# Tonanguyxiro/FastBN

Hardware: AMD Instinct MI355X
Metric: JT test-cases/sec (ALARM, Munin) + PC-stable CI-tests/sec, 1/2/4/8 GPU (higher is better)
Workload: dtype f64

## Files before the change

### fastbn_amd/csrc/jt_codegen.cpp

```cpp
#include <algorithm>
#include <map>
#include <cstdio>
#include <cstdlib>
#include <functional>
#include <sstream>
#include <string>

#include "fbn_internal.h"

namespace fbn {

namespace {

int LocOfT(const Table &t, int v) {
    for (size_t i = 0; i < t.vars.size(); ++i)
        if (t.vars[i] == v) return (int)i;
    return -1;
}

std::string Lit(double x) {
    char b[64];
    snprintf(b, sizeof b, "%.17g", x);
    std::string s = b;
    if (s.find_first_of(".eEn") == std::string::npos) s += ".0";
    return s;
}

}

bool JTCodegenEligible(const JTPlanHost &plan, int64_t *entry_ops) {
    int64_t tmax = 0, ops = 0;
    for (const auto &t : plan.cliques) {
        tmax = std::max<int64_t>(tmax, t.size());
        ops += t.size() * (4 + (int64_t)t.vars.size());
    }
    if (entry_ops) *entry_ops = ops;
    for (int d : plan.dom)
        if (d > 32) return false;
    return tmax <= 256 && ops <= 40000;
}

namespace {

class JTGen {
  public:
    JTGen(const JTPlanHost &p, bool fast_order, bool var_major) : plan(p), fast(fast_order), vmajor(var_major) {}
    int Run(std::string &src, int64_t *wave_entries, std::vector<double> &initv);
    int64_t lds_rows = 0;
    int64_t pool_rows = 0;
    JTPlacement place;
    bool iv_lds = false;

  private:
    const JTPlanHost &plan;
    const bool fast;
    const bool vmajor;
    std::ostringstream o;
    std::vector<int> okw_word, okw_pos, out_off;
    std::vector<int64_t> sep_row, init_off;
    std::vector<std::vector<int>> cand;
    std::vector<int> home;
    std::vector<int> msep;
    std::vector<int> mclq;
    void MargTerms(int v, const std::vector<std::vector<std::string>> &terms);
    int nobs = 0;
    bool profile = false;
    static constexpr int64_t kInitBatch = 16;
    bool in_merged = false;
    int min_waves = 1;
    bool marg_v2 = true;
    std::vector<std::vector<std::string>> col_loc, dis_loc;
    std::vector<bool> md_reg;
    std::vector<bool> leaf_rc, col_store;
    void LoadCol(const std::string &name, int s) {
        if (!leaf_rc[s]) return Load(name, s);
        const int c = plan.sep_down[s];
        const int64_t Ts = plan.seps[s].size(), Q = plan.cliques[c].size() / Ts;
        for (int64_t j = 0; j < Ts; ++j) o << "        double " << name << s << "_" << j << ";\n";
        o << "        { // recompute the Collect message of leaf clique " << c << "\n";
        const std::string P = "r" + name;
        InitProd(P, c, {}, -1, "");
        for (int64_t j = 0; j < Ts; ++j) {
            std::vector<std::string> terms;
            for (int64_t q = 0; q < Q; ++q) terms.push_back(N(P, c, q * Ts + j));
            o << "        " << name << s << "_" << j << " = " << TreeSum(terms) << ";\n";
        }
        o << "        }\n";
    }
    void PlaceMessages(const std::vector<int> &post, const std::vector<int> &pre, int64_t budget, int64_t reg_cap,
                       bool quiet);
    static constexpr int64_t kRegFile = 256, kRegSlackVM = 16, kRegSlackCM = 32, kDefaultRegPool = kRegFile;
    int64_t peak_need = 0;
    std::vector<int64_t> reg_extra;
    std::vector<std::string> reg_names;
    std::string B(int k) const {
        return profile ? "        FBN_OP_BOUNDARY(); FBN_STAMP(" + std::to_string(k) + ");\n" : "        FBN_OP_BOUNDARY();\n";
    }

    std::string R(int c) const {
        std::vector<unsigned> m(nobs, 0u);
        for (int v : plan.cliques[c].vars) m[v / 32] |= 1u << (v % 32);
        std::ostringstream t;
        t << "(" << plan.cliques[c].vars.size();
        for (int k = 0; k < nobs; ++k)
            if (m[k]) t << " - __builtin_popcount(obs" << k << " & " << m[k] << "u)";
        t << ")";
        return t.str();
    }
    std::string observed(int v) const {
        std::ostringstream t;
        t << "((obs" << v / 32 << " >> " << v % 32 << ") & 1u)";
        return t.str();
    }
    int child(int s) const { return plan.sep_down[s]; }
    int64_t SepIndex(const Table &t, const Table &sp, int64_t e) const {
        int64_t r = e, idx = 0;
        for (size_t j = 0; j < t.vars.size(); ++j) {
            const int64_t dgt = r / t.cum[j];
            r %= t.cum[j];
            const int l = LocOfT(sp, t.vars[j]);
            if (l >= 0) idx += dgt * sp.cum[l];
        }
        return idx;
    }
    void Init(const std::string &P, int c);
    void InitProd(const std::string &P, int c, const std::vector<std::pair<int, std::string>> &kids, int up,
                  const std::string &upM);
    void Mul(const std::string &P, int c, int s, const std::string &M);
    void SepCol(const std::string &P, int c, int s, bool store);
    void DMul(const std::string &P, int c, int s, const std::string &M);
    void SepDis(const std::string &P, int c, int s, const std::string &old, bool store);
    void Marg(const std::string &P, int c);
    void Load(const std::string &name, int s) {
        const auto &loc = name == "ld" ? dis_loc[s] : col_loc[s];
        for (int64_t j = 0; j < plan.seps[s].size(); ++j)
            o << "        const double " << name << s << "_" << j << " = " << loc[j] << ";\n";
    }
    static constexpr int64_t kRegEntries = 144;
    std::string N(const std::string &P, int c, int64_t e) const {
        if (e >= kRegEntries) return "L(" + std::to_string(e - kRegEntries) + ")";
        return P + std::to_string(c) + "_" + std::to_string(e);
    }
    bool normed = false;
    std::string Val(const std::string &P, int c, int64_t e) const {
        return (normed || fast) ? N(P, c, e) : "dv(" + N(P, c, e) + ", den, y)";
    }
    static std::string TreeSum(const std::vector<std::string> &t, size_t b, size_t e) {
        if (e - b == 1) return t[b];
        const size_t m = b + (e - b) / 2;
        return "(" + TreeSum(t, b, m) + " + " + TreeSum(t, m, e) + ")";
    }
    static std::string TreeSum(const std::vector<std::string> &t) { return TreeSum(t, 0, t.size()); }
    void Normalize(const std::string &P, int c) {
        const Table &t = plan.cliques[c];
        for (int64_t e = 0; e < t.size(); ++e) o << (e % 8 ? " " : (e ? "\n        " : "        ")) << N(P, c, e) << " = dv(" << N(P, c, e) << ", den, y);";
        o << "\n" << B(6);
        normed = true;
    }
};

void JTGen::Init(const std::string &P, int c) {
    const Table &t = plan.cliques[c];
    const int nv = (int)t.vars.size();
    std::vector<bool> ev_here(nv, true);
    for (int j = 0; j < nv; ++j) ev_here[j] = !fast || home[t.vars[j]] == c;
    for (int j = 0; j < nv; ++j) {
        const int v = t.vars[j];
        if (!ev_here[j]) continue;
        for (int d = 0; d < plan.dom[v]; ++d)
            o << (d ? " " : "        ") << "const bool k" << P << c << "_" << j << "_" << d << " = (okw" << okw_word[v] << " >> "
              << okw_pos[v] + d << ") & 1u;";
        o << "\n";
    }
    if (!fast) o << "        double s_" << P << c << " = 0.0;\n";
    const int64_t kB = 16, T = t.size();
    auto loads = [&](int64_t b0) {
        if (b0 >= T) return;
        o << "       ";
        for (int64_t e = b0; e < std::min(T, b0 + kB); ++e)
            o << " const double w" << P << c << "_" << e << " = IV(" << init_off[c] + e << ");";
        o << "\n        __builtin_amdgcn_sched_barrier(0);\n";
    };
    loads(0);
    for (int64_t b0 = 0; b0 < T; b0 += kB) {
        loads(b0 + kB);
        for (int64_t e = b0; e < std::min(T, b0 + kB); ++e) {
            std::ostringstream cond;
            int64_t r = e;
            bool any = false;
            for (int j = 0; j < nv; ++j) {
                const int64_t dgt = r / t.cum[j];
                r %= t.cum[j];
                if (!ev_here[j]) continue;
                cond << (any ? " && " : "") << "k" << P << c << "_" << j << "_" << dgt;
                any = true;
            }
            o << "        " << (e < kRegEntries ? "double " : "") << N(P, c, e) << " = ";
            if (any) o << "sel(" << cond.str() << ", w" << P << c << "_" << e << ");";
            else o << "w" << P << c << "_" << e << ";";
            if (!fast) o << " s_" << P << c << " += " << N(P, c, e) << ";";
            o << "\n";
        }
        o << "        __builtin_amdgcn_sched_barrier(0);\n";
    }
    if (!fast) o << "        den = s_" << P << c << "; y = 1.0 / den; bad |= den_bad(den);\n";
    o << B(2);
    normed = false;
}

void JTGen::InitProd(const std::string &P, int c, const std::vector<std::pair<int, std::string>> &kids, int up,
                     const std::string &upM) {
    const Table &t = plan.cliques[c];
    const int nv = (int)t.vars.size();
    std::vector<bool> ev_here(nv, false);
    for (int j = 0; j < nv; ++j) ev_here[j] = home[t.vars[j]] == c;
    for (int j = 0; j < nv; ++j) {
        if (!ev_here[j]) continue;
        const int v = t.vars[j];
        for (int d = 0; d < plan.dom[v]; ++d)
            o << (d ? " " : "        ") << "const double i" << P << c << "_" << j << "_" << d << " = (double)((okw"
              << okw_word[v] << " >> " << okw_pos[v] + d << ") & 1u);";
        o << "\n";
    }
    std::vector<std::vector<int64_t>> kidx(kids.size());
    for (size_t i = 0; i < kids.size(); ++i) {
        const Table &sp = plan.seps[kids[i].first];
        for (int64_t e = 0; e < t.size(); ++e) kidx[i].push_back(SepIndex(t, sp, e));
    }
    const int64_t Tup = up >= 0 ? plan.seps[up].size() : 0;
    const int64_t kB = kInitBatch, T = t.size();
    auto loads = [&](int64_t b0) {
        if (b0 >= T) return;
        o << "       ";
        for (int64_t e = b0; e < std::min(T, b0 + kB); ++e)
            o << " const double w" << P << c << "_" << e << " = IV(" << init_off[c] + e << ");";
        o << "\n        __builtin_amdgcn_sched_barrier(0);\n";
    };
    loads(0);
    for (int64_t b0 = 0; b0 < T; b0 += kB) {
        loads(b0 + kB);
        for (int64_t e = b0; e < std::min(T, b0 + kB); ++e) {
            std::vector<std::string> f{"w" + P + std::to_string(c) + "_" + std::to_string(e)};
            int64_t r = e;
            for (int j = 0; j < nv; ++j) {
                const int64_t dgt = r / t.cum[j];
                r %= t.cum[j];
                if (ev_here[j]) f.push_back("i" + P + std::to_string(c) + "_" + std::to_string(j) + "_" + std::to_string(dgt));
            }
            for (size_t i = 0; i < kids.size(); ++i)
                f.push_back(kids[i].second + std::to_string(kids[i].first) + "_" + std::to_string(kidx[i][e]));
            if (up >= 0) f.push_back(upM + std::to_string(up) + "_" + std::to_string(e % Tup));
            std::function<std::string(size_t, size_t)> prod = [&](size_t lo, size_t hi) -> std::string {
                if (hi - lo == 1) return f[lo];
                const size_t m = lo + (hi - lo) / 2;
                return "(" + prod(lo, m) + " * " + prod(m, hi) + ")";
            };
            o << "        " << (e < kRegEntries ? "double " : "") << N(P, c, e) << " = " << prod(0, f.size()) << ";\n";
        }
        o << "        __builtin_amdgcn_sched_barrier(0);\n";
    }
    o << B(2);
    normed = false;
}

void JTGen::Mul(const std::string &P, int c, int s, const std::string &M) {
    const Table &t = plan.cliques[c], &sp = plan.seps[s];
    std::vector<std::vector<int64_t>> inv(sp.size());
    for (int64_t e = 0; e < t.size(); ++e) inv[SepIndex(t, sp, e)].push_back(e);
    for (int64_t j = 0; j < sp.size(); ++j) {
        o << "       ";
        for (int64_t e : inv[j]) o << " " << N(P, c, e) << " = " << Val(P, c, e) << " * " << M << s << "_" << j << ";";
        o << "\n";
    }
    if (!fast) {
        o << "        { double sm = 0.0;";
        for (int64_t e = 0; e < t.size(); ++e) o << " sm += " << N(P, c, e) << ";";
        o << " den = sm; y = 1.0 / den; bad |= den_bad(den); }\n";
    }
    o << B(3);
    normed = false;
}

void JTGen::SepCol(const std::string &P, int c, int s, bool store) {
    const Table &t = plan.cliques[c];
    const int64_t Ts = plan.seps[s].size(), Q = t.size() / Ts;
    if (fast) {
        for (int64_t j = 0; j < Ts; ++j) {
            std::vector<std::string> terms;
            for (int64_t q = 0; q < Q; ++q) terms.push_back(N(P, c, q * Ts + j));
            o << "        const double mc" << s << "_" << j << " = " << TreeSum(terms) << ";";
            if (store) o << " " << col_loc[s][j] << " = mc" << s << "_" << j << ";";
            o << "\n";
        }
        if (!in_merged) o << B(4);
        return;
    }
    for (int64_t j = 0; j < Ts; ++j) {
        o << "        const double mc" << s << "_" << j << " = " << Val(P, c, j);
        for (int64_t q = 1; q < Q; ++q) o << " + " << Val(P, c, q * Ts + j);
        o << ";";
        if (store) o << " " << col_loc[s][j] << " = mc" << s << "_" << j << ";";
        o << "\n";
    }
    o << B(4);
}

void JTGen::DMul(const std::string &P, int c, int s, const std::string &M) {
    const Table &t = plan.cliques[c];
    const int64_t Ts = plan.seps[s].size();
    for (int64_t j = 0; j < Ts; ++j) {
        o << "       ";
        for (int64_t e = j; e < t.size(); e += Ts)
            o << " " << N(P, c, e) << " = " << Val(P, c, e) << " * " << M << s << "_" << j << ";";
        o << "\n";
    }
    if (!fast) {
        o << "        { double sm = 0.0;";
        for (int64_t e = 0; e < t.size(); ++e) o << " sm += " << N(P, c, e) << ";";
        o << " den = sm; y = 1.0 / den; bad |= den_bad(den); }\n";
    }
    o << B(5);
    normed = false;
}

void JTGen::SepDis(const std::string &P, int c, int s, const std::string &old, bool store) {
    const Table &t = plan.cliques[c], &sp = plan.seps[s];
    std::vector<std::vector<int64_t>> lists(sp.size());
    for (int64_t e = 0; e < t.size(); ++e) lists[SepIndex(t, sp, e)].push_back(e);
    if (fast) {
        for (int64_t j = 0; j < sp.size(); ++j) {
            std::vector<std::string> terms;
            for (int64_t e : lists[j]) terms.push_back(N(P, c, e));
            const std::string sa = "sa" + std::to_string(s) + "_" + std::to_string(j);
            o << "        const double " << sa << " = " << TreeSum(terms) << ";";
            o << " double md" << s << "_" << j << "; { const double od = " << old << s << "_" << j
              << "; const double q = " << sa << " * frcp(od); md" << s << "_" << j << " = (od == 0.0) ? 0.0 : q; }";
            if (store) o << " " << dis_loc[s][j] << " = md" << s << "_" << j << ";";
            o << "\n";
        }
        for (size_t l = 0; l < sp.vars.size(); ++l) {
            const int v = sp.vars[l];
            if (msep[v] != s) continue;
            std::vector<std::vector<std::string>> terms(plan.dom[v]);
            for (int64_t j = 0; j < sp.size(); ++j)
                terms[(j / sp.cum[l]) % sp.dims[l]].push_back("sa" + std::to_string(s) + "_" + std::to_string(j));
            MargTerms(v, terms);
        }
        if (!in_merged) o << B(7);
        return;
    }
    for (int64_t j = 0; j < sp.size(); ++j) {
        o << "        double md" << s << "_" << j << ";";
        o << " { double a = " << Val(P, c, lists[j][0]) << ";";
        for (size_t q = 1; q < lists[j].size(); ++q) o << " a += " << Val(P, c, lists[j][q]) << ";";
        o << " const double od = " << old << s << "_" << j << "; md" << s << "_" << j << " = (od == 0.0) ? 0.0 : a / od; }";
        if (store) o << " " << dis_loc[s][j] << " = md" << s << "_" << j << ";";
        o << "\n";
    }
    o << B(7);
}

void JTGen::MargTerms(int v, const std::vector<std::vector<std::string>> &terms) {
    const int dim = plan.dom[v];
    if (marg_v2) {
        o << "        { // marginal of var " << v << "\n          const bool ob = " << observed(v) << " != 0u;\n";
        std::vector<std::string> ps;
        for (int d = 0; d < dim; ++d) {
            o << "          const double p" << d << " = " << TreeSum(terms[d]) << ";\n";
            ps.push_back("p" + std::to_string(d));
        }
        o << "          const double tot = " << TreeSum(ps) << "; const double yt = frcp(tot); bad |= ob ? 0u : den_bad(tot);\n";
        if (v == 0) {
            o << "          if (ACT && !ob) { int lab = 0; double mp = 0.0, m2 = 0.0;";
            for (int d = 0; d < dim; ++d)
                o << " { const double q = dv(p" << d << ", tot, yt); if (q > mp) { m2 = mp; mp = q; lab = " << d
                  << "; } else if (q > m2) m2 = q; }";
            o << " labels[CS] = lab; bad |= (mp - m2 <= 1e-12 * mp) ? 1u : 0u; }\n";
        }
        for (int d = 0; d < dim; ++d) {
            const int64_t k = out_off[v] + d;
            if (marg_v2 && d + 1 < dim) {
                o << "          if (ACT) OUTS2(" << k << ", ob ? 0.0 : dv(p" << d << ", tot, yt), ob ? 0.0 : dv(p" << d + 1 << ", tot, yt));\n";
                ++d;
            } else {
                o << "          if (ACT) OUTS(" << k << ", ob ? 0.0 : dv(p" << d << ", tot, yt));\n";
            }
        }
        o << "        }\n";
        return;
    }
    o << "        if (!" << observed(v) << ") { // marginal of var " << v << "\n";
    std::vector<std::string> ps;
    for (int d = 0; d < dim; ++d) {
        o << "          const double p" << d << " = " << TreeSum(terms[d]) << ";\n";
        ps.push_back("p" + std::to_string(d));
    }
    o << "          const double tot = " << TreeSum(ps) << "; const double yt = frcp(tot); bad |= den_bad(tot);\n";
    if (v == 0) {
        o << "          if (ACT) { int lab = 0; double mp = 0.0, m2 = 0.0;";
        for (int d = 0; d < dim; ++d)
            o << " { const double q = dv(p" << d << ", tot, yt); if (q > mp) { m2 = mp; mp = q; lab = " << d
              << "; } else if (q > m2) m2 = q; }";
        o << " labels[CS] = lab; bad |= (mp - m2 <= 1e-12 * mp) ? 1u : 0u; }\n";
    }
    o << "          if (ACT) {";
    for (int d = 0; d < dim; ++d) o << " OUTS(" << out_off[v] + d << ", dv(p" << d << ", tot, yt));";
    o << " }\n        }\n";
}

void JTGen::Marg(const std::string &P, int c) {
    const Table &t = plan.cliques[c];
    for (size_t j = 0; j < t.vars.size(); ++j) {
        const int v = t.vars[j];
        const int dim = plan.dom[v];
        const int64_t cum = t.cum[j], bw = dim * cum, nhi = t.size() / bw;
        if (fast) {
            if (mclq[v] != c || msep[v] >= 0) continue;
            std::vector<std::vector<std::string>> terms(dim);
            for (int d = 0; d < dim; ++d)
                for (int64_t hi = 0; hi < nhi; ++hi)
                    for (int64_t l = 0; l < cum; ++l) terms[d].push_back(N(P, c, hi * bw + d * cum + l));
            MargTerms(v, terms);
            if (!in_merged) o << B(8);
            continue;
        } else {
            o << "        { int b = " << R(cand[v][0]) << ", sl = " << cand[v][0] << ";";
            for (size_t k = 1; k < cand[v].size(); ++k)
                o << " { const int r = " << R(cand[v][k]) << "; if (r < b) { b = r; sl = " << cand[v][k] << "; } }";
            o << "\n        if (sl == " << c << " && !" << observed(v) << ") { // marginal of var " << v << "\n";
        }
        if (fast) {
            std::vector<std::string> ps;
            for (int d = 0; d < dim; ++d) {
                std::vector<std::string> terms;
                for (int64_t hi = 0; hi < nhi; ++hi)
                    for (int64_t l = 0; l < cum; ++l) terms.push_back(N(P, c, hi * bw + d * cum + l));
                o << "          const double p" << d << " = " << TreeSum(terms) << ";\n";
                ps.push_back("p" + std::to_string(d));
            }
            o << "          const double tot = " << TreeSum(ps) << "; const double yt = frcp(tot); bad |= den_bad(tot);\n";
// ... 182 lines not shown
    for (int i : byst) {
        const Item &it = items[i];
        for (size_t k = 0; k < active.size();) {
            if (items[active[k]].b < it.a) {
                for (int64_t r : rows_of[active[k]]) free_rows.push_back(r);
                std::sort(free_rows.rbegin(), free_rows.rend());
                active.erase(active.begin() + k);
            } else {
                ++k;
            }
        }
        for (int64_t j = nreg[i]; j < it.n; ++j) {
            rows_of[i].push_back(free_rows.back());
            pool_rows = std::max<int64_t>(pool_rows, free_rows.back() + 1);
            free_rows.pop_back();
        }
        active.push_back(i);
    }
    col_loc.assign(ns, {});
    dis_loc.assign(ns, {});
    sep_row.assign(ns, -1);
    reg_names.clear();
    std::vector<int64_t> sep_skip(ns, 0);
    for (int s = 0; s < ns; ++s) sep_skip[s] = plan.seps[s].size();
    for (size_t i = 0; i < items.size(); ++i)
        if (!in_lds[i]) sep_skip[items[i].s] = std::min(sep_skip[items[i].s], nreg[i]);
    int64_t grow = 0;
    place = JTPlacement();
    for (size_t i = 0; i < items.size(); ++i) {
        const Item &it = items[i];
        auto &loc = it.dist ? dis_loc[it.s] : col_loc[it.s];
        loc.assign(it.n, std::string());
        for (int64_t j = 0; j < nreg[i]; ++j) {
            loc[j] = (it.dist ? "rd" : "rc") + std::to_string(it.s) + "_" + std::to_string(j);
            reg_names.push_back(loc[j]);
        }
        place.reg[it.dist] += nreg[i];
        if (in_lds[i]) {
            for (int64_t j = nreg[i]; j < it.n; ++j) loc[j] = "LP(" + std::to_string(rows_of[i][j - nreg[i]]) + ")";
            place.lds[it.dist] += it.n - nreg[i];
            continue;
        }
        if (nreg[i] == it.n) continue;
        if (sep_row[it.s] < 0) sep_row[it.s] = grow, grow += it.n - sep_skip[it.s];
        for (int64_t j = nreg[i]; j < it.n; ++j) loc[j] = "W(" + std::to_string(sep_row[it.s] + j - sep_skip[it.s]) + "LL)";
        place.global[it.dist] += it.n - nreg[i];
    }
    place.workspace_rows = grow;
    place.lds_pool_rows = pool_rows;
    for (int s = 0; s < ns; ++s) {
        if (sep_row[s] < 0) sep_row[s] = 0;
        if (dis_loc[s].empty()) dis_loc[s].assign(plan.seps[s].size(), "0.0");
        if (col_loc[s].empty()) col_loc[s].assign(plan.seps[s].size(), "0.0");
    }
    if (!quiet && KnobSet("FBN_JT_PLACE_DEBUG")) {
        int64_t leaf = 0;
        for (int s = 0; s < ns; ++s)
            if (plan.clique_down[plan.sep_down[s]].empty()) leaf += plan.seps[s].size();
        fprintf(stderr, "placement: pool %lld of %lld rows; Collect rows LDS %lld global %lld; Distribute rows LDS %lld "
                        "global %lld (registers: the rest); global rows %lld; leaf-separator rows %lld\n",
                (long long)pool_rows, (long long)cap, (long long)place.lds[0], (long long)place.global[0],
                (long long)place.lds[1], (long long)place.global[1], (long long)grow, (long long)leaf);
        if (reg_cap > 0)
            fprintf(stderr, "register pool (cap %lld rows): Collect rows %lld, Distribute rows %lld\n", (long long)reg_cap,
                    (long long)place.reg[0], (long long)place.reg[1]);
        std::string u;
        for (int t = 0; t <= 2 * nc; ++t) u += std::to_string(use[t]) + (t == nc - 1 ? " | " : " ");
        fprintf(stderr, "pool rows in use by time (Collect | Distribute): %s\n", u.c_str());
        if (fast) {
            std::string m;
            for (int v = 0; v < (int)plan.dom.size(); ++v) {
                const int t = msep[v] >= 0 ? nc + pi[plan.sep_up[msep[v]]] : nc + pi[mclq[v]];
                m += std::to_string(v) + ":" + std::to_string(t) + " ";
            }
            fprintf(stderr, "marginal time per variable: %s\n", m.c_str());
        }
    }
}

int JTGen::Run(std::string &src, int64_t *wave_entries, std::vector<double> &initv) {
    const int nc = (int)plan.cliques.size(), ns = (int)plan.seps.size(), V = plan.num_nodes;
    profile = KnobOr("FBN_JT_PROFILE", 0) != 0;
    marg_v2 = fast && KnobOr("FBN_JT_MARG_V2", 1) != 0;
    lds_rows = 0;
    for (const auto &t : plan.cliques) lds_rows = std::max<int64_t>(lds_rows, t.size() - kRegEntries);
    initv.clear();
    init_off.assign(nc, 0);
    for (int c = 0; c < nc; ++c) {
        init_off[c] = (int64_t)initv.size();
        initv.insert(initv.end(), plan.cliques[c].pot.begin(), plan.cliques[c].pot.end());
    }
    int SD = 0;
    out_off.assign(V, 0);
    for (int v = 0; v < V; ++v) out_off[v] = SD, SD += plan.dom[v];
    cand.assign(V, {});
    for (int c = 0; c < nc; ++c)
        for (int v : plan.cliques[c].vars) cand[v].push_back(c);
    home.assign(V, -1);
    for (int v = 0; v < V; ++v)
        for (int q : cand[v])
            if (home[v] < 0 || plan.cliques[q].size() < plan.cliques[home[v]].size()) home[v] = q;
    msep.assign(V, -1);
    if (fast)
        for (int sp = 0; sp < ns; ++sp)
            for (int v : plan.seps[sp].vars) {
                const int64_t have = msep[v] >= 0 ? plan.seps[msep[v]].size() : plan.cliques[home[v]].size();
                if (plan.seps[sp].size() < have) msep[v] = sp;
            }
    mclq = home;
    std::vector<int64_t> weight(nc, 0);
    {
        std::function<int64_t(int)> w = [&](int c) {
            weight[c] = plan.cliques[c].size();
            for (int s : plan.clique_down[c]) weight[c] += w(child(s));
            return weight[c];
        };
        for (int r : plan.roots) w(r);
    }
    auto dfs = [&](bool collect, int visit, std::vector<int> &post_o, std::vector<int> &pre_o) {
        std::vector<std::vector<int>> kids(nc);
        for (int c = 0; c < nc; ++c) {
            kids[c] = plan.clique_down[c];
            if (visit)
                std::stable_sort(kids[c].begin(), kids[c].end(), [&](int x, int y) {
                    return visit == 1 ? weight[child(x)] > weight[child(y)] : weight[child(x)] < weight[child(y)];
                });
        }
        std::vector<int> roots = plan.roots;
        if (!collect) std::reverse(roots.begin(), roots.end());
        std::vector<std::pair<int, size_t>> st;
        size_t next_root = 0;
        while (!st.empty() || next_root < roots.size()) {
            if (st.empty()) st.push_back({roots[next_root++], 0});
            auto &top = st.back();
            const int c = top.first;
            if (top.second == 0) pre_o.push_back(c);
            if (top.second < kids[c].size()) {
                const int ch = child(kids[c][top.second++]);
                st.push_back({ch, 0});
            } else {
                post_o.push_back(c);
                st.pop_back();
            }
        }
    };
    std::vector<int> post, pre, unused;
    dfs(true, 0, post, unused);
    unused.clear();
    dfs(false, 0, unused, pre);
    if ((int)post.size() != nc) return SetError(FBN_ERR_LIMIT, "codegen: tree traversal covers %zu of %d cliques", post.size(), nc);
    const int64_t kBudget = fast ? 260 : 200;
    int64_t reg_cap = fast && vmajor ? kDefaultRegPool : 0;
    if (const char *e = KnobValue("FBN_JT_REG_POOL")) reg_cap = fast ? std::max(0, atoi(e)) : 0;
    if (reg_cap > 0) {
        int64_t best = -1, plan_peak = 0;
        int bvc = 0, bvd = 0;
        std::vector<int> bpost = post, bpre = pre;
        for (int vc = 0; vc < 3; ++vc)
            for (int vd = 0; vd < 3; ++vd) {
                std::vector<int> po, pr, un;
                dfs(true, vc, po, un);
                un.clear();
                dfs(false, vd, un, pr);
                PlaceMessages(po, pr, kBudget, reg_cap, true);
                if (best < 0) plan_peak = peak_need;
                else if (peak_need > plan_peak) continue;
                const int64_t g = place.global[0] + place.global[1];
                if (best < 0 || g < best) best = g, bpost = po, bpre = pr, bvc = vc, bvd = vd;
            }
        post = bpost, pre = bpre;
        if (KnobSet("FBN_JT_PLACE_DEBUG"))
            fprintf(stderr, "child order (0 plan, 1 heaviest subtree first, 2 last): Collect %d, Distribute %d\n", bvc, bvd);
    }
    PlaceMessages(post, pre, kBudget, reg_cap, false);
    int64_t rows = 0;
    for (int s = 0; s < ns; ++s) rows = std::max<int64_t>(rows, sep_row[s] + plan.seps[s].size());
    *wave_entries = std::max<int64_t>(rows, 1);

    o << "// generated by libfastbn (jt_codegen.cpp): " << nc << " cliques, " << ns << " separators, "
      << (fast ? "fast" : "exact") << " arithmetic order\n";
    o << "#define FBN_V " << V << "\n#define FBN_SD " << SD << "\n#define FBN_WE " << *wave_entries << "LL\n";
    o << "#define FBN_LP_BASE " << lds_rows << "\n";
    o << "#define FBN_IV_BASE " << (lds_rows + pool_rows) * 64 << "\n#define FBN_NIV " << initv.size() << "\n";
    o << "#define FBN_IV_LDS " << (iv_lds ? 1 : 0) << "\n#define FBN_MIN_WAVES " << min_waves << "\n";
    if (vmajor) o << "#define FBN_VMAJOR 1\n";
    o << R"FBN(typedef signed char i8;
__device__ __forceinline__ double dv(double x, double den, double y) {  // x / den (Markstein, see jt_kernels.hip)
    const double q = x * y;
    const double r = __builtin_fma(-den, q, x);
    return __builtin_fma(r, y, q);
}
// row r of the per-wave workspace, this lane: uniform row base (SGPRs) + lane byte offset (VGPR)
typedef __attribute__((address_space(1))) double gdouble;
typedef __attribute__((address_space(1))) char gchar;
typedef __attribute__((address_space(4))) const double cdouble;
#define W(row) (*(gdouble *)((gchar *)(Wb + (row) * 64) + (unsigned long long)lo))
// LDS row of the clique in flight (entries beyond the register-resident part of large tables)
typedef __attribute__((address_space(3))) double ldouble;
extern __shared__ double fbn_lds[];
#define L(row) (ltail[(row) * 64])
// LDS message pool row (after the clique tail)
#define LP(row) (ltail[(FBN_LP_BASE + (row)) * 64])
// initial potentials: copied into LDS once per wave (wave-uniform address: broadcast reads), or
// read with scalar loads from the constant buffer
#if FBN_IV_LDS
#define IV(k) (ivl[k])
#else
#define IV(k) (ivc[k])
#endif
// unconditional (LDS broadcast) load + select: no branch per table entry
__device__ __forceinline__ double sel(bool c, double v) { return c ? v : 0.0; }
#define FBN_STAMP(k) do { unsigned long long t_; __asm__ volatile("s_memtime %0\n\ts_waitcnt lgkmcnt(0)" : "=s"(t_) :: "memory"); pacc[k] += t_ - tprev; tprev = t_; } while (0)
__device__ __forceinline__ unsigned den_bad(double d) { return (d >= 0x1p-600 && d <= 0x1p+600) ? 0u : 1u; }
// fast order: 1 / x as v_rcp_f64 + one Newton step (relative error <= 2.3e-15 over 2^-60..2^60,
// tools/micro/fp64_ilp.hip), branch-free, so independent reciprocals overlap; the operands are
// range-checked by den_bad (a block outside [2^-600, 2^600] goes to the exact pass)
__device__ __forceinline__ double frcp(double x) {
    const double r = __builtin_amdgcn_rcp(x);
    return __builtin_fma(r, __builtin_fma(-x, r, 1.0), r);
}
// this lane's case / output row, recomputed per segment from the (laundered) block index
#define CS (blkl * 64 + lane)
#define ACT (CS < ncases)
#ifdef FBN_VMAJOR
// variable-major output [SD][ncases]: value k of every case is one column, so a store instruction
// writes 64 consecutive cases = 512 contiguous bytes (4 full lines) instead of one value into 64
// lines.  Through a buffer resource: voffset = the lane's case (bytes), soffset = column k (bytes,
// (The host takes this kernel only when ncases * SD * 8 < 2^31.)
typedef unsigned fbn_u2v __attribute__((ext_vector_type(2)));
#ifdef FBN_NO_OUT
#define OUTS(k, v) do { if (ncases < 0) __builtin_amdgcn_raw_buffer_store_b64(__builtin_bit_cast(fbn_u2v, (double)(v)), mrs, (int)(CS * 8), (int)(k) * mcb, 0); } while (0)
#else
#define OUTS(k, v) __builtin_amdgcn_raw_buffer_store_b64(__builtin_bit_cast(fbn_u2v, (double)(v)), mrs, (int)(CS * 8), (int)(k) * mcb, 0)
#endif
#else
#define OUT(k) (marg[CS * FBN_SD + (k)])
#ifdef FBN_NO_OUT  // diagnostic only (FBN_JT_NO_OUT=1): marginals computed, never stored
#define OUTS(k, v) do { if (ncases < 0) OUT(k) = (v); } while (0)
#else
#define OUTS(k, v) (OUT(k) = (v))
#endif
#endif
#ifdef FBN_VMAJOR
#define OUTS2(k, a, b) do { OUTS(k, a); OUTS((k) + 1, b); } while (0)
#else
// two adjacent output values in one 16-byte store (8-byte aligned: the rows are 8 * FBN_SD bytes)
typedef double fbn_d2u __attribute__((ext_vector_type(2), aligned(8)));
#ifdef FBN_NO_OUT
#define OUTS2(k, a, b) do { if (ncases < 0) *(fbn_d2u *)&OUT(k) = (fbn_d2u){(a), (b)}; } while (0)
#else
#define OUTS2(k, a, b) (*(fbn_d2u *)&OUT(k) = (fbn_d2u){(a), (b)})
#endif
#endif
extern "C" __global__ void __launch_bounds__(64, FBN_MIN_WAVES)
fbn_jt_gen(const i8 *__restrict__ evid, double *__restrict__ marg, int *__restrict__ labels,
           double *__restrict__ ws, int *__restrict__ flags, const double *ivp, long long ncases,
           unsigned long long *__restrict__ prof) {
    const int lane = threadIdx.x;
    // LDS bases are laundered at every op boundary (so addresses fold into ds_* offsets instead of
    // being hoisted as loop-invariant constants)
    ldouble *ltail = (ldouble *)fbn_lds + lane;
#if FBN_IV_LDS
    ldouble *ivl = (ldouble *)fbn_lds + FBN_IV_BASE;
    for (int k = lane; k < FBN_NIV; k += 64) IV(k) = ivp[k];
    __syncthreads();
#else
    const cdouble *ivc = (const cdouble *)ivp;
    ldouble *ivl = (ldouble *)fbn_lds;  // unused (laundered at op boundaries)
#endif
    unsigned long long pacc[10] = {0, 0, 0, 0, 0, 0, 0, 0, 0, 0}, tprev = __builtin_amdgcn_s_memtime();
#ifdef FBN_WS_FOLD
    gdouble *Wb = (gdouble *)ws + (unsigned long long)(blockIdx.x % FBN_WS_FOLD) * FBN_WE * 64;
#else
    gdouble *Wb = (gdouble *)ws + (unsigned long long)blockIdx.x * FBN_WE * 64;
#endif
    unsigned lo = (unsigned)lane * 8;
#ifdef FBN_VMAJOR
    const __amdgpu_buffer_rsrc_t mrs = __builtin_amdgcn_make_buffer_rsrc(marg, 0, 0x7FFFFFFF, 0x00020000);
    const int mcb = (int)ncases * 8;  // column stride, bytes
#endif
    for (long long blk = blockIdx.x; blk * 64 < ncases; blk += gridDim.x) {
        long long blkl = blk;
        const long long cs = blk * 64 + lane;
        const long long csr = cs < ncases ? cs : ncases - 1;
        const i8 *__restrict__ ev = evid + csr * FBN_V;
        unsigned bad = 0u;  // laundered at op boundaries: checked where computed, never deferred
        double den, y;
)FBN";
    okw_word.assign(V, 0);
    okw_pos.assign(V, 0);
    int nokw = 0;
    {
        int pos = 32;
        for (int v = 0; v < V; ++v) {
            if (pos + plan.dom[v] > 32) ++nokw, pos = 0;
            okw_word[v] = nokw - 1, okw_pos[v] = pos, pos += plan.dom[v];
        }
    }
    nobs = (V + 31) / 32;
    {
        std::vector<std::string> regs;
        for (int k = 0; k < nokw; ++k) regs.push_back("okw" + std::to_string(k));
        for (int k = 0; k < nobs; ++k) regs.push_back("obs" + std::to_string(k));
        o << "#define FBN_OP_BOUNDARY() do { __asm__ volatile(\"\" : \"+s\"(Wb), \"+v\"(lo), \"+v\"(ltail), \"+v\"(ivl), \"+v\"(bad), \"+s\"(blkl) :: \"memory\");";
        for (size_t i = 0; i < regs.size(); i += 16) {
            o << " __asm__ volatile(\"\" :";
            for (size_t k = i; k < std::min(regs.size(), i + 16); ++k) o << (k > i ? ", " : " ") << "\"+v\"(" << regs[k] << ")";
            o << ");";
        }
        o << " __builtin_amdgcn_sched_barrier(0); } while (0)\n";
    }
    for (int k = 0; k < nokw; ++k) o << "        unsigned okw" << k << " = 0u;\n";
    for (int k = 0; k < nobs; ++k) o << "        unsigned obs" << k << " = 0u;\n";
    for (size_t i = 0; i < reg_names.size(); i += 8) {
        o << "        double";
        for (size_t k = i; k < std::min(reg_names.size(), i + 8); ++k) o << (k > i ? ", " : " ") << reg_names[k];
        o << ";\n";
    }
    for (int v = 0; v < V; ++v) {
        const unsigned full = (plan.dom[v] >= 32) ? 0xFFFFFFFFu : ((1u << plan.dom[v]) - 1u);
        o << "        { const int x = ev[" << v << "]; okw" << okw_word[v] << " |= (x < 0 ? " << full << "u : (1u << x)) << "
          << okw_pos[v] << "; obs" << v / 32 << " |= (x >= 0 ? 1u : 0u) << " << v % 32 << "; }\n";
    }
    o << B(0);

    auto tsize = [&](int c) { return plan.cliques[c].size(); };
    auto collect_loads = [&](size_t k, std::vector<int> &ls) {
        ls.clear();
        const int c = post[k];
        const auto &down = plan.clique_down[c];
        for (size_t i = 0; i < down.size(); ++i)
            if (!(k > 0 && child(down[i]) == post[k - 1])) ls.push_back(down[i]);
    };
    auto rows_of = [&](const std::vector<int> &ls) {
        int64_t r = 0;
        for (int s : ls) r += plan.seps[s].size();
        return r;
    };
    const int cont_root = post.back() == pre.front() ? pre.front() : -1;
    std::vector<bool> loaded_a(ns, false);
    for (size_t k = 0; k < post.size(); ++k) {
        const int c = post[k];
        if (plan.clique_up[c] < 0 && c != cont_root) continue;
        std::vector<int> mine, next;
        collect_loads(k, mine);
        o << "        // ---- collect clique " << c << " (" << tsize(c) << " entries)\n";
        for (int s : mine)
            if (!loaded_a[s]) Load("la", s), loaded_a[s] = true;
        const bool next_runs = k + 1 < post.size() && (plan.clique_up[post[k + 1]] >= 0 || post[k + 1] == cont_root);
        if (next_runs) {
            collect_loads(k + 1, next);
            int64_t pend = 0;
            for (int s : mine) pend += plan.seps[s].size();
            if (tsize(c) + pend + rows_of(next) + reg_extra[k] <= kBudget)
                for (int s : next)
                    if (!loaded_a[s]) Load("la", s), loaded_a[s] = true;
        }
        o << B(1);
        const auto &down = plan.clique_down[c];
        if (fast) {
            std::vector<std::pair<int, std::string>> kids;
            for (int s : down) kids.push_back({s, loaded_a[s] ? "la" : "mc"});
            InitProd("t", c, kids, -1, "");
        } else {
            Init("t", c);
            for (size_t i = 0; i < down.size(); ++i) {
                const int s = down[i];
                Mul("t", c, s, loaded_a[s] ? "la" : "mc");
            }
        }
        if (c != cont_root) SepCol("t", c, plan.clique_up[c], col_store[plan.clique_up[c]]);
    }
    auto kids_rows = [&](int c) {
        int64_t r = 0;
        for (int s : plan.clique_down[c]) r += plan.seps[s].size();
        return r;
    };
    auto early_lb = [&](int c) {
        const int up = plan.clique_up[c];
        const int64_t held = (up >= 0) ? plan.seps[up].size() : 0;
        return tsize(c) + kids_rows(c) + held <= kBudget;
    };
    std::vector<bool> loaded_b(ns, false), loaded_d(ns, false);
    for (size_t k = 0; k < pre.size(); ++k) {
        const int c = pre[k];
        const int up = plan.clique_up[c];
        const bool early = early_lb(c);
        o << "        // ---- distribute clique " << c << " (" << tsize(c) << " entries)\n";
        int64_t pend = 0;
        if (early)
            for (int s : plan.clique_down[c]) {
                if (!loaded_b[s]) LoadCol("lb", s), loaded_b[s] = true;
                pend += plan.seps[s].size();
            }
        if (up >= 0 && md_reg[up]) pend += plan.seps[up].size();
        if (k + 1 < pre.size()) {
            const int nx = pre[k + 1], nup = plan.clique_up[nx];
            const bool ld_next = nup >= 0 && !md_reg[nup] && plan.sep_up[nup] != c;
            const int64_t nrows = (early_lb(nx) ? kids_rows(nx) : 0) + (ld_next ? plan.seps[nup].size() : 0);
            if (tsize(c) + pend + nrows + reg_extra[nc + k] <= kBudget) {
                if (early_lb(nx))
                    for (int s : plan.clique_down[nx])
                        if (!loaded_b[s] && !leaf_rc[s]) Load("lb", s), loaded_b[s] = true;
                if (ld_next && !loaded_d[nup]) Load("ld", nup), loaded_d[nup] = true;
            }
        }
        o << B(1);
        std::string P = "t";
        if (c != cont_root && fast && early) {
            P = "u";
            if (up >= 0 && !md_reg[up] && !loaded_d[up]) Load("ld", up), loaded_d[up] = true, o << B(1);
            std::vector<std::pair<int, std::string>> kids;
            for (int s : plan.clique_down[c]) kids.push_back({s, "lb"});
            InitProd(P, c, kids, up, up < 0 ? "" : md_reg[up] ? "md" : "ld");
        } else if (c != cont_root) {
            P = "u";
            Init(P, c);
            for (int s : plan.clique_down[c]) {
                if (!early) LoadCol("lb", s), o << B(1);
                Mul(P, c, s, "lb");
            }
            if (up >= 0) {
                if (!md_reg[up] && !loaded_d[up]) Load("ld", up), loaded_d[up] = true, o << B(1);
                DMul(P, c, up, md_reg[up] ? "md" : "ld");
            }
        }
        const auto &down = plan.clique_down[c];
        if (!fast && down.size() + plan.cliques[c].vars.size() >= 2) Normalize(P, c);
        in_merged = fast && early;
        for (size_t i = 0; i < down.size(); ++i) {
            if (!early) LoadCol("lc", down[i]), o << B(1);
            SepDis(P, c, down[i], early ? "lb" : "lc", !md_reg[down[i]]);
        }
        Marg(P, c);
        if (in_merged) o << B(8);
        in_merged = false;
    }
    if (marg_v2) o << "        if (ACT && " << observed(0) << ") labels[CS] = 0;\n";
    for (int v = 0; v < V && !marg_v2; ++v) {
        o << "        if (ACT && " << observed(v) << ") {";
        for (int d = 0; d < plan.dom[v]; ++d) o << " OUTS(" << out_off[v] + d << ", 0.0);";
        if (v == 0) o << " labels[CS] = 0;";
        o << " }\n";
    }
    o << R"(        const bool any_bad = __builtin_amdgcn_ballot_w64(bad != 0u) != 0ull;
        if (lane == 0) flags[blk] = any_bad ? 1 : 0;  // every block writes its flag: no clearing pass
    }
    if (prof && lane == 0)
        for (int k = 0; k < 10; ++k) prof[(unsigned long long)blockIdx.x * 16 + k] = pacc[k];
}
)";
    src = o.str();
    return FBN_OK;
}

}

int GenerateJTKernel(const JTPlanHost &plan, std::string &src, int64_t *wave_entries, std::vector<double> &initv,
                     int64_t *lds_bytes, bool fast, bool var_major, JTPlacement *placement) {
    JTGen g(plan, fast, var_major);
    int rc = g.Run(src, wave_entries, initv);
    if (placement) *placement = g.place;
    if (lds_bytes) *lds_bytes = ((g.lds_rows + g.pool_rows) * 64 + (g.iv_lds ? (int64_t)initv.size() : 0)) * 8;
    return rc;
}

}
```

### fastbn_amd/csrc/knobs.h

```cpp
#ifndef FBN_KNOBS_H
#define FBN_KNOBS_H

#include <algorithm>
#include <cstdint>
#include <cstdlib>
#include <cstring>
#include <thread>

namespace fbn {

enum KnobKind { kSeam, kDiagnostic, kLocation };
enum KnobRead { kPerCall, kOnce, kOutside };

struct Knob {
    const char *name;
    const char *dflt;
    KnobKind kind;
    KnobRead read;
};

inline constexpr Knob kKnobs[] = {
    {"FBN_CI_BITSN", "off: levels >= 2 count from byte columns", kSeam, kPerCall},
    {"FBN_CI_FORCE_BITS", "off: bit-sliced columns from 4096 samples", kSeam, kPerCall},
    {"FBN_CI_GRAM4_SPLITS", "CUs / tiles", kSeam, kPerCall},
    {"FBN_CI_GRAM_NO_MFMA", "off: FP4 MFMA Gram where it pays", kSeam, kPerCall},
    {"FBN_CI_NO_BAND", "off: the G^2 decision band is built", kSeam, kPerCall},
    {"FBN_CI_NO_BITS", "off", kSeam, kPerCall},
    {"FBN_CI_NO_DER2", "off", kSeam, kPerCall},
    {"FBN_CI_NO_GRAM", "off", kSeam, kPerCall},
    {"FBN_CI_NO_PACK2", "off", kSeam, kPerCall},
    {"FBN_CI_NO_PAIRS", "off", kSeam, kPerCall},
    {"FBN_CI_NO_ZEROCOPY", "off", kSeam, kPerCall},
    {"FBN_CI_PACK2", "off: packed columns from 65536 samples", kSeam, kPerCall},
    {"FBN_JT_LDS_POOL", "the LDS left beside the kernel's own", kSeam, kPerCall},
    {"FBN_JT_LEAF_RC", "0", kSeam, kPerCall},
    {"FBN_JT_MARG_V2", "1", kSeam, kPerCall},
    {"FBN_JT_REG_POOL", "the registers left under the budget", kSeam, kPerCall},
    {"FBN_JT_TILING", "0", kSeam, kPerCall},
    {"FBN_JT_TW", "1", kSeam, kPerCall},
    {"FBN_PC_DIST_FORCE_EXCHANGE", "off", kSeam, kOutside},
    {"FBN_PC_FULLSPEC", "16384", kSeam, kPerCall},
    {"FBN_PC_GEN_GENERAL", "off", kSeam, kPerCall},
    {"FBN_PC_GROWTH", "4 (host rounds), 2 (device level 1)", kSeam, kPerCall},
    {"FBN_PC_HOST_L0L1", "off", kSeam, kPerCall},
    {"FBN_PC_HOST_L1", "off", kSeam, kPerCall},
    {"FBN_PC_L0CHUNK", "4194304", kSeam, kPerCall},
    {"FBN_PC_L1CAP", "524288", kSeam, kPerCall},
    {"FBN_PC_L1_MAXCHUNK", "65536", kSeam, kPerCall},
    {"FBN_PC_NO_MISCREEN", "off", kSeam, kPerCall},
    {"FBN_PC_NO_SMALL", "off", kSeam, kPerCall},
    {"FBN_PC_PIPELINE_EDGES", "kPipelineEdges", kSeam, kPerCall},
    {"FBN_PC_ROUND0", "8192", kSeam, kPerCall},
    {"FBN_PC_SMALL_COOP", "unset: cooperative launch where it fits", kSeam, kPerCall},
    {"FBN_PC_SMALL_FAIL", "unset", kSeam, kPerCall},
    {"FBN_JT_PLACE_DEBUG", "off", kDiagnostic, kPerCall},
    {"FBN_JT_PROFILE", "0", kDiagnostic, kPerCall},
    {"FBN_JT_VDEBUG", "0", kDiagnostic, kPerCall},
    {"FBN_PC_SMALL_TRACE", "off", kDiagnostic, kOnce},
    {"FBN_PC_TIMING", "off", kDiagnostic, kOnce},
    {"FBN_PLAN_TIMING", "off", kDiagnostic, kOnce},
    {"FBN_KERNEL_CACHE", "fastbn_amd/kcache beside the library", kLocation, kPerCall},
    {"FBN_LIB_PATH", "libfastbn.so beside the package", kLocation, kOutside},
    {"OMP_NUM_THREADS", "min(16, hardware threads)", kLocation, kPerCall},
};

inline const char *KnobValue(const char *name) {
    for (const Knob &k : kKnobs)
        if (!strcmp(k.name, name)) return getenv(name);
    abort();
}

inline bool KnobSet(const char *name) { return KnobValue(name) != nullptr; }

inline int64_t KnobOr(const char *name, int64_t dflt) {
    const char *v = KnobValue(name);
    return v ? atoll(v) : dflt;
}

inline bool PcTiming() {
    static const bool on = KnobSet("FBN_PC_TIMING");
    return on;
}

inline int HostThreads() {
    const unsigned hc = std::thread::hardware_concurrency();
    int t = (int)std::max(1u, std::min(16u, hc ? hc : 1u));
    if (const char *e = KnobValue("OMP_NUM_THREADS")) t = std::max(1, std::min(t, atoi(e)));
    return t;
}

}

#endif
```

### fastbn_amd/prebuild.py

```python
import os
import tempfile

from . import api, synth

REPO = os.path.dirname(os.path.dirname(os.path.abspath(__file__)))
ALARM_XML = os.path.join(REPO, "tests", "golden", "alarm", "alarm.xml")
SYNTH_SMALL = dict(n=60, seed=5, window=6)


def synth_small_xml(dirname):
    path = os.path.join(dirname, "synth60.xml")
    synth.random_network(SYNTH_SMALL["n"], seed=SYNTH_SMALL["seed"], window=SYNTH_SMALL["window"], path=path)
    return path


def prebuild(xml_paths, layouts=(0,)):
    out = []
    for xml in xml_paths:
        jt = api.JunctionTree(api.Network(xml), device=-1)
        if jt.info["specialized_eligible"]:
            for layout in layouts:
                jt.set_output_layout(layout)
                for exact in (None, True):
                    jt.set_exact(exact)
                    out.append(jt.build_kernel())
    return out


def fixture_xmls(dirname):
    import glob
    import gzip
    out = []
    for gz in sorted(glob.glob(os.path.join(REPO, "tests", "golden", "synth_nets", "*.xml.gz"))):
        path = os.path.join(dirname, os.path.basename(gz)[:-3])
        with gzip.open(gz, "rb") as f, open(path, "wb") as g:
            g.write(f.read())
        out.append(path)
    return out


def _load_tests_module(name):
    import importlib.util
    import sys
    spec = importlib.util.spec_from_file_location(name, os.path.join(REPO, "tests", name + ".py"))
    mod = importlib.util.module_from_spec(spec)
    keep, sys.dont_write_bytecode = sys.dont_write_bytecode, True
    try:
        spec.loader.exec_module(mod)
    finally:
        sys.dont_write_bytecode = keep
    return mod


def count_map_nets():
    J = _load_tests_module("jt_nets")
    return [(J.conflict_net(*J.CONFLICT_FORMS["xmlbif"]), (0,)), (J.conflict_net(*J.CONFLICT_FORMS["counts"]), (0, 1)),
            (J.counts_net(J.COUNTS_SEED, "small"), (0,)), (J.counts_net(J.COUNTS_SEED, "dom32"), (0,))]


def prebuild_forests(dirname):
    N = _load_tests_module("jt_forest_nets")
    out = []
    jf = api.JunctionForest(api.Network.from_counts(*N.disconnected()), device=-1)
    for layout in (0, 1):
        jf.set_output_layout(layout)
        for exact in (None, True):
            jf.set_exact(exact)
            out.append(jf.build_kernel())
    star = N.star_net()
    path = os.path.join(dirname, "forest.xml")
    synth.random_network(path=path, **N.RANDOM)
    for net in (api.Network.from_counts(star.dims, star.parents, star.counts), api.Network(path)):
        out.append(api.JunctionForest(net, device=-1).build_kernel())
    return out


def prebuild_count_maps():
    out = []
    for net, layouts in count_map_nets():
        jt = api.JunctionTree(api.Network.from_counts(net.dims, net.parents, net.counts), device=-1)
        assert jt.info["specialized_eligible"]
        for layout in layouts:
            jt.set_output_layout(layout)
            for exact in (None, True):
                jt.set_exact(exact)
                out.append(jt.build_kernel())
    return out


ALARM_TEST_OPTIONS = ({"FBN_JT_LEAF_RC": "1"}, {"FBN_JT_LDS_POOL": "0"}, {"FBN_JT_MARG_V2": "0"},
                      {"FBN_JT_REG_POOL": "0"}, {"FBN_JT_REG_POOL": "256"})


def prebuild_options(xml, options, layout=0):
    import subprocess
    import sys
    out = []
    for opt in options:
        env = dict(os.environ, **opt)
        code = ("import sys; sys.path.insert(0, %r); from fastbn_amd import api; "
                "jt = api.JunctionTree(api.Network(%r), device=-1); jt.set_output_layout(%d); "
                "print(jt.build_kernel())" % (REPO, xml, layout))
        r = subprocess.run([sys.executable, "-c", code], env=env, capture_output=True, text=True, check=True)
        out.append(r.stdout.strip().splitlines()[-1])
    return out


def prebuild_default(clean=True):
    with tempfile.TemporaryDirectory() as d:
        built = prebuild([ALARM_XML], layouts=(0, 1)) + prebuild([synth_small_xml(d)] + fixture_xmls(d))
        built += prebuild_forests(d)
    built += prebuild_options(ALARM_XML, ALARM_TEST_OPTIONS)
    built += prebuild_options(ALARM_XML, ({"FBN_JT_REG_POOL": "0"}, {"FBN_JT_REG_POOL": "256"}), layout=1)
    built += prebuild_count_maps()
    if clean:
        keep = {os.path.basename(p) for p in built}
        kdir = os.path.join(REPO, "fastbn_amd", "kcache")
        for f in os.listdir(kdir) if os.path.isdir(kdir) else []:
            if f.endswith(".hsaco") and f not in keep:
                os.remove(os.path.join(kdir, f))
    return built
```

Before: 969.2 million.

## Pipeline potential loads and emit level-wise product/sum trees in JT codegen

```diff
diff --git a/fastbn_amd/csrc/jt_codegen.cpp b/fastbn_amd/csrc/jt_codegen.cpp
--- a/fastbn_amd/csrc/jt_codegen.cpp
+++ b/fastbn_amd/csrc/jt_codegen.cpp
@@ -66,6 +66,27 @@
     int nobs = 0;
     bool profile = false;
     static constexpr int64_t kInitBatch = 16;
+    static constexpr int64_t kSchedFirst = 8;
+    bool sched = false;
+    int64_t BatchEnd(int64_t b0, int64_t T) const { return std::min(T, b0 + (b0 == 0 && sched ? kSchedFirst : kInitBatch)); }
+    bool iv_issued = false;
+    static constexpr int64_t kSchedGroup = 2;
+    int64_t ntemp = 0;
+    struct LTree {
+        std::string head;
+        std::vector<std::string> leaves;
+        std::string tail;
+    };
+    std::vector<std::string> Levels(const std::vector<LTree> &trees, char op);
+    bool in_leaf_rc = false;
+    std::string IvLoads(const std::string &P, int c, int64_t b0);
+    std::vector<std::string> iv_first;
+    void IvFirst(const std::string &P, int c) {
+        if (iv_first.empty()) o << IvLoads(P, c, 0);
+        else iv_first.back() = IvLoads(P, c, 0);
+        iv_issued = true;
+    }
+    static std::string IvMarker(size_t n) { return "/*@iv" + std::to_string(n) + "@*/"; }
     bool in_merged = false;
     int min_waves = 1;
     bool marg_v2 = true;
@@ -79,7 +100,9 @@
         for (int64_t j = 0; j < Ts; ++j) o << "        double " << name << s << "_" << j << ";\n";
         o << "        { // recompute the Collect message of leaf clique " << c << "\n";
         const std::string P = "r" + name;
+        in_leaf_rc = true;
         InitProd(P, c, {}, -1, "");
+        in_leaf_rc = false;
         for (int64_t j = 0; j < Ts; ++j) {
             std::vector<std::string> terms;
             for (int64_t q = 0; q < Q; ++q) terms.push_back(N(P, c, q * Ts + j));
@@ -208,6 +231,58 @@
     normed = false;
 }
 
+std::vector<std::string> JTGen::Levels(const std::vector<LTree> &trees, char op) {
+    std::vector<std::string> lv;
+    const std::string ops = std::string(" ") + op + " ";
+    for (const LTree &t : trees) {
+        std::function<std::pair<std::string, size_t>(size_t, size_t)> node = [&](size_t lo, size_t hi) -> std::pair<std::string, size_t> {
+            if (hi - lo == 1) return {t.leaves[lo], 0};
+            const size_t m = lo + (hi - lo) / 2;
+            const auto a = node(lo, m), b = node(m, hi);
+            const size_t h = 1 + std::max(a.second, b.second);
+            if (lv.size() < h) lv.resize(h);
+            if (lo == 0 && hi == t.leaves.size()) {
+                lv[h - 1] += t.head + a.first + ops + b.first + ";" + t.tail;
+                return {"", h};
+            }
+            const std::string nm = "x" + std::to_string(ntemp++);
+            lv[h - 1] += "        const double " + nm + " = " + a.first + ops + b.first + ";\n";
+            return {nm, h};
+        };
+        const auto r = node(0, t.leaves.size());
+        if (t.leaves.size() == 1) {
+            if (lv.empty()) lv.resize(1);
+            lv[0] += t.head + r.first + ";" + t.tail;
+        }
+    }
+    return lv;
+}
+
+std::string JTGen::IvLoads(const std::string &P, int c, int64_t b0) {
+    const int64_t T = plan.cliques[c].size();
+    std::ostringstream o;
+    if (b0 >= T) return std::string();
+    const int64_t b1 = BatchEnd(b0, T);
+    if (sched && !iv_lds) {
+        for (int64_t e = b0, n = 16; e < b1; e += n) {
+            while (n > b1 - e) n /= 2;
+            const std::string wv = "wv" + P + std::to_string(c) + "_" + std::to_string(e);
+            o << "        const " << (n > 1 ? "fbn_w" + std::to_string(n) : std::string("double")) << " " << wv << " = *(const volatile "
+              << (n > 1 ? "fbn_cw" + std::to_string(n) : std::string("cdouble")) << " *)&IV(" << init_off[c] + e << ");";
+            for (int64_t k = 0; k < n; ++k)
+                o << " const double w" << P << c << "_" << e + k << " = " << wv << (n > 1 ? "[" + std::to_string(k) + "]" : std::string()) << ";";
+            o << "\n";
+        }
+        o << "        __builtin_amdgcn_sched_barrier(0);\n";
+        return o.str();
+    }
+    o << "       ";
+    for (int64_t e = b0; e < b1; ++e)
+        o << " const double w" << P << c << "_" << e << " = IV(" << init_off[c] + e << ");";
+    o << "\n        __builtin_amdgcn_sched_barrier(0);\n";
+    return o.str();
+}
+
 void JTGen::InitProd(const std::string &P, int c, const std::vector<std::pair<int, std::string>> &kids, int up,
                      const std::string &upM) {
     const Table &t = plan.cliques[c];
@@ -228,28 +303,45 @@
         for (int64_t e = 0; e < t.size(); ++e) kidx[i].push_back(SepIndex(t, sp, e));
     }
     const int64_t Tup = up >= 0 ? plan.seps[up].size() : 0;
-    const int64_t kB = kInitBatch, T = t.size();
-    auto loads = [&](int64_t b0) {
-        if (b0 >= T) return;
-        o << "       ";
-        for (int64_t e = b0; e < std::min(T, b0 + kB); ++e)
-            o << " const double w" << P << c << "_" << e << " = IV(" << init_off[c] + e << ");";
-        o << "\n        __builtin_amdgcn_sched_barrier(0);\n";
+    const int64_t T = t.size();
+    if (!iv_issued) o << IvLoads(P, c, 0);
+    iv_issued = false;
+    auto factors = [&](int64_t e) {
+        std::vector<std::string> f{"w" + P + std::to_string(c) + "_" + std::to_string(e)};
+        int64_t r = e;
+        for (int j = 0; j < nv; ++j) {
+            const int64_t dgt = r / t.cum[j];
+            r %= t.cum[j];
+            if (ev_here[j]) f.push_back("i" + P + std::to_string(c) + "_" + std::to_string(j) + "_" + std::to_string(dgt));
+        }
+        for (size_t i = 0; i < kids.size(); ++i)
+            f.push_back(kids[i].second + std::to_string(kids[i].first) + "_" + std::to_string(kidx[i][e]));
+        if (up >= 0) f.push_back(upM + std::to_string(up) + "_" + std::to_string(e % Tup));
+        return f;
     };
-    loads(0);
-    for (int64_t b0 = 0; b0 < T; b0 += kB) {
-        loads(b0 + kB);
-        for (int64_t e = b0; e < std::min(T, b0 + kB); ++e) {
-            std::vector<std::string> f{"w" + P + std::to_string(c) + "_" + std::to_string(e)};
-            int64_t r = e;
-            for (int j = 0; j < nv; ++j) {
-                const int64_t dgt = r / t.cum[j];
-                r %= t.cum[j];
-                if (ev_here[j]) f.push_back("i" + P + std::to_string(c) + "_" + std::to_string(j) + "_" + std::to_string(dgt));
-            }
-            for (size_t i = 0; i < kids.size(); ++i)
-                f.push_back(kids[i].second + std::to_string(kids[i].first) + "_" + std::to_string(kidx[i][e]));
-            if (up >= 0) f.push_back(upM + std::to_string(up) + "_" + std::to_string(e % Tup));
+    const std::string wpre = "w" + P + std::to_string(c) + "_";
+    for (int64_t b0 = 0, b1; b0 < T && sched; b0 = b1) {
+        b1 = BatchEnd(b0, T);
+        bool pending = b1 < T;
+        for (int64_t e0 = b0; e0 < b1; e0 += kSchedGroup) {
+            std::vector<LTree> trees;
+            for (int64_t e = e0; e < std::min(b1, e0 + kSchedGroup); ++e)
+                trees.push_back({"        " + std::string(e < kRegEntries ? "double " : "") + N(P, c, e) + " = ", factors(e), "\n"});
+            for (const std::string &l : Levels(trees, '*')) {
+                o << l;
+                if (pending && l.find(wpre) != std::string::npos) {
+                    o << "        __builtin_amdgcn_sched_barrier(0);\n" << IvLoads(P, c, b1);
+                    pending = false;
+                }
+            }
+        }
+        o << "        __builtin_amdgcn_sched_barrier(0);\n";
+    }
+    for (int64_t b0 = 0, b1; b0 < T && !sched; b0 = b1) {
+        b1 = BatchEnd(b0, T);
+        o << IvLoads(P, c, b1);
+        for (int64_t e = b0; e < b1; ++e) {
+            const std::vector<std::string> f = factors(e);
             std::function<std::string(size_t, size_t)> prod = [&](size_t lo, size_t hi) -> std::string {
                 if (hi - lo == 1) return f[lo];
                 const size_t m = lo + (hi - lo) / 2;
@@ -260,6 +352,7 @@
         o << "        __builtin_amdgcn_sched_barrier(0);\n";
     }
     o << B(2);
+    if (sched && !in_leaf_rc) o << IvMarker(iv_first.size()) << "\n", iv_first.push_back(std::string());
     normed = false;
 }
 
@@ -285,7 +378,17 @@
     const Table &t = plan.cliques[c];
     const int64_t Ts = plan.seps[s].size(), Q = t.size() / Ts;
     if (fast) {
-        for (int64_t j = 0; j < Ts; ++j) {
+        for (int64_t j0 = 0; j0 < Ts && sched; j0 += kSchedGroup) {
+            std::vector<LTree> trees;
+            for (int64_t j = j0; j < std::min(Ts, j0 + kSchedGroup); ++j) {
+                const std::string mc = "mc" + std::to_string(s) + "_" + std::to_string(j);
+                std::vector<std::string> terms;
+                for (int64_t q = 0; q < Q; ++q) terms.push_back(N(P, c, q * Ts + j));
+                trees.push_back({"        const double " + mc + " = ", terms, (store ? " " + col_loc[s][j] + " = " + mc + ";" : std::string()) + "\n"});
+            }
+            for (const std::string &l : Levels(trees, '+')) o << l;
+        }
+        for (int64_t j = 0; j < Ts && !sched; ++j) {
             std::vector<std::string> terms;
             for (int64_t q = 0; q < Q; ++q) terms.push_back(N(P, c, q * Ts + j));
             o << "        const double mc" << s << "_" << j << " = " << TreeSum(terms) << ";";
@@ -774,6 +877,7 @@
     const int64_t kBudget = fast ? 260 : 200;
     int64_t reg_cap = fast && vmajor ? kDefaultRegPool : 0;
     if (const char *e = KnobValue("FBN_JT_REG_POOL")) reg_cap = fast ? std::max(0, atoi(e)) : 0;
+    sched = reg_cap > 0 && KnobOr("FBN_JT_SCHED", 1) != 0;
     if (reg_cap > 0) {
         int64_t best = -1, plan_peak = 0;
         int bvc = 0, bvd = 0;
@@ -932,6 +1036,10 @@
         }
         o << " __builtin_amdgcn_sched_barrier(0); } while (0)\n";
     }
+    if (sched)
+        for (int n = 2; n <= 16; n *= 2)
+            o << "        typedef double fbn_w" << n << " __attribute__((ext_vector_type(" << n << "), aligned(8)));"
+              << " typedef __attribute__((address_space(4))) fbn_w" << n << " fbn_cw" << n << ";\n";
     for (int k = 0; k < nokw; ++k) o << "        unsigned okw" << k << " = 0u;\n";
     for (int k = 0; k < nobs; ++k) o << "        unsigned obs" << k << " = 0u;\n";
     for (size_t i = 0; i < reg_names.size(); i += 8) {
@@ -978,6 +1086,7 @@
                 for (int s : next)
                     if (!loaded_a[s]) Load("la", s), loaded_a[s] = true;
         }
+        if (fast && sched) IvFirst("t", c);
         o << B(1);
         const auto &down = plan.clique_down[c];
         if (fast) {
@@ -1027,6 +1136,7 @@
                 if (ld_next && !loaded_d[nup]) Load("ld", nup), loaded_d[nup] = true;
             }
         }
+        if (c != cont_root && fast && early && sched) IvFirst("u", c);
         o << B(1);
         std::string P = "t";
         if (c != cont_root && fast && early) {
@@ -1073,6 +1183,10 @@
 }
 )";
     src = o.str();
+    for (size_t n = 0; n < iv_first.size(); ++n) {
+        const size_t at = src.find(IvMarker(n) + "\n");
+        src.replace(at, IvMarker(n).size() + 1, iv_first[n]);
+    }
     return FBN_OK;
 }
 
diff --git a/fastbn_amd/csrc/knobs.h b/fastbn_amd/csrc/knobs.h
--- a/fastbn_amd/csrc/knobs.h
+++ b/fastbn_amd/csrc/knobs.h
@@ -36,6 +36,7 @@
     {"FBN_JT_LEAF_RC", "0", kSeam, kPerCall},
     {"FBN_JT_MARG_V2", "1", kSeam, kPerCall},
     {"FBN_JT_REG_POOL", "the registers left under the budget", kSeam, kPerCall},
+    {"FBN_JT_SCHED", "1: the potentials' load pipeline and level-wise products (read only with the register pool on)", kSeam, kPerCall},
     {"FBN_JT_TILING", "0", kSeam, kPerCall},
     {"FBN_JT_TW", "1", kSeam, kPerCall},
     {"FBN_PC_DIST_FORCE_EXCHANGE", "off", kSeam, kOutside},
diff --git a/fastbn_amd/prebuild.py b/fastbn_amd/prebuild.py
--- a/fastbn_amd/prebuild.py
+++ b/fastbn_amd/prebuild.py
@@ -92,6 +92,10 @@
                       {"FBN_JT_REG_POOL": "0"}, {"FBN_JT_REG_POOL": "256"})
 
 
+SCHED_TEST_OPTIONS = {0: ({"FBN_JT_REG_POOL": "256"}, {"FBN_JT_REG_POOL": "256", "FBN_JT_SCHED": "0"}),
+                      1: ({}, {"FBN_JT_SCHED": "0"})}
+
+
 def prebuild_options(xml, options, layout=0):
     import subprocess
     import sys
@@ -110,7 +114,10 @@
     with tempfile.TemporaryDirectory() as d:
         built = prebuild([ALARM_XML], layouts=(0, 1)) + prebuild([synth_small_xml(d)] + fixture_xmls(d))
         built += prebuild_forests(d)
+        built += prebuild_options(synth_small_xml(d), SCHED_TEST_OPTIONS[1], layout=1)
     built += prebuild_options(ALARM_XML, ALARM_TEST_OPTIONS)
+    for layout in (0, 1):
+        built += prebuild_options(ALARM_XML, SCHED_TEST_OPTIONS[layout], layout=layout)
     built += prebuild_options(ALARM_XML, ({"FBN_JT_REG_POOL": "0"}, {"FBN_JT_REG_POOL": "256"}), layout=1)
     built += prebuild_count_maps()
     if clean:
```

Result: faster. 982.7 million, median of 6 (+1.4%).
